# dojo-sim/ContactImplicitMPC.jl

Hardware: AMD Instinct MI355X
Metric: MPC steps/s (quadruped, H=40, fp64) (higher is better)
Workload: dtype f64

## Files before the change

contactimplicitmpc/jl_amd/csrc/cimpc_host.cpp:

```cpp
#include <hip/hip_runtime.h>

#include <algorithm>
#include <chrono>
#include <cmath>
#include <cstdio>
#include <cstdlib>
#include <cstring>
#include <string>
#include <vector>

#include "cimpc_internal.h"
#include "lin_table.h"
#include "newton_state.h"
#include "schedule_plan.h"

using namespace cimpc;

namespace {

thread_local std::string g_create_error;

enum ProfClass { PC_IP = 0, PC_KKT = 1, PC_RESID = 2, PC_OTHER = 3, PC_ASYNC = 4, PC_COUNT = 5 };

struct ProfRec {
// ... 220 lines not shown
    (void)hipStreamSynchronize(h->stream);
    if (h->rs.st) (void)hipStreamSynchronize(h->rs.st);
    if (h->rs.st_kkt) (void)hipStreamSynchronize(h->rs.st_kkt);
    for (auto& r : h->prof_recs) {
        float ms = 0.f;
        if (hipEventElapsedTime(&ms, r.a, r.b) == hipSuccess) {
            h->prof_ms[r.cls] += ms;
            h->prof_n[r.cls] += 1;
        }
        h->ev_pool.push_back(r.a);
        h->ev_pool.push_back(r.b);
    }
    h->prof_recs.clear();
}

IpParams make_ip_params(cimpc_ctx* h, const TrajDev& T, int par, int* pending_counter, double* zout) {
    IpParams p{};
    p.tab = h->d_tab;
    p.Q = h->Q;
    p.Q.par = par;
    p.wpk = h->sched.wpk;
    p.q = T.q;
    p.theta = T.th;
    p.gam = T.g;
    p.bfr = T.b;
    p.alt = h->alt_set ? h->d_alt : nullptr;
    p.d = h->S.d;
    p.dz = h->S.dz;
    p.nu = nullptr; p.dtn = nullptr; p.dtn_ld = h->S.dtn_ld;
    p.status = h->S.ip_status;
    p.iters = h->S.ip_iters;
    p.zout = zout;
    p.pflag = h->S.pflag;
    p.pstate = h->d_pstate;
    p.pending_count = pending_counter;
    p.iter_cap = h->kn.sched.iter_cap;
    p.slots = CS;
    p.H = h->dm.H;
    p.o = h->ip;
    p.kc_floor = h->ip.kappa_tol / h->ip.undercut;
    p.tau_floor = 1.0 - h->ip.eps_min;
    p.reg_floor = h->ip.kappa_tol * h->ip.gamma_reg;
    p.budget_ticks = h->ip_budget_ticks;
    p.generic_static = h->kn.generic_static ? 1 : 0;
    return p;
}

int run_sweep(cimpc_ctx* h, int par, int* pending_counter, double* zout, hipStream_t st, int iter_cap = 0, int* drain_counter = nullptr,
              bool with_products = false, long long hint = -1) {
    IpParams p = make_ip_params(h, h->S.cand, par, pending_counter, zout);
    if (with_products && h->S.dtn != nullptr) { p.nu = h->S.nu_cand; p.dtn = h->S.dtn; }
    if (iter_cap > 0) p.iter_cap = iter_cap;
    const SweepLaunch l = plan_sweep(h->kn.sched, h->sched, hint, p.iter_cap, h->ip.max_iter, drain_counter != nullptr);
    p.wpk = l.wpk; p.direct = l.direct;
    if (l.drain_thresh > 0) { p.drain_count = drain_counter; p.drain_thresh = l.drain_thresh; p.drain_min = h->kn.sched.drain_min; }
    prof_begin(h, PC_IP, st);
    int rc = launch_ip_sweep(&h->dm, p, l.waves, st);
    prof_end(h, st);
    if (rc != CIMPC_OK) return fail(h, rc, "ip sweep launch failed");
    return CIMPC_OK;
}

static void set_kkt_backend(cimpc_ctx* h) {
    NewtonDev& S = h->S;
    KktCaps& c = h->kc;
    c.cfg = h->dm.mode == CIMPC_MODE_CONFIGURATION;
    c.velocity = S.V != nullptr;
    c.cf_tiny = h->cf_tiny;
    c.wide_tiles = (h->dm.nq > 16 || h->dm.nu > 16) && h->dm.nq <= 24 && h->dm.nu <= 24;
    c.condensed = kkt_condensed_available(S);
    c.mfma = kkt_mfma_available(S);
    c.packed = kkt_packed_available(S);
    c.twisted = kkt_twisted_available(S);
    c.duo = kkt_duo_available(S);
    c.mixed = kkt_mixed_available(S);
    auto pick_band_form = [&](auto avail) {
        for (int r = h->band_reduce_ok ? 1 : 0; r >= 0; --r) { S.band_reduce = r; if (avail()) return true; }
        S.band_reduce = h->band_reduce_ok ? 1 : 0;
        return false;
    };
    S.band_reduce = h->band_reduce_ok ? 1 : 0;
    c.banded = c.cfg && pick_band_form([&] { return kkt_banded_available(S); });
    c.cf_reduce = !c.cfg && (c.velocity ? pick_band_form([&] { return kkt_cf_reduce_available(S); }) : kkt_cf_reduce_available(S));
    c.banded_twisted = kkt_banded_twisted_available(c.cfg ? S : cf_shadow(S));
    h->kb = select_kkt_backend(c, h->nt.kkt_backend);
    S.good_src = kkt_lazy_commit(h->kp, c, h->kb) ? h->d_good_src : nullptr;
}

int ensure_kkt_ws(cimpc_ctx* h) {
    if (h->kb == KktBackend::Condensed) return CIMPC_OK;
    if (h->kb == KktBackend::CondensedMixed) {
        if (h->d_mix_ws) return CIMPC_OK;
        if (dev_alloc(h, &h->d_mix_ws, kkt_mixed_workspace_doubles(h->S)) != CIMPC_OK) return CIMPC_ERR_HIP;
        return dev_alloc(h, &h->d_mix_nfb, 1);
    }
    const bool cf = h->kb == KktBackend::CfCondensed || h->kb == KktBackend::CfBanded;
    if (cf && !h->d_cf_ws && dev_alloc(h, &h->d_cf_ws, cf_reduce_doubles(h->S)) != CIMPC_OK) return CIMPC_ERR_HIP;
    if (h->kb == KktBackend::CfCondensed) return CIMPC_OK;
    const size_t need = cf ? kkt_dense_workspace_doubles(cf_shadow(h->S), true) : kkt_dense_workspace_doubles(h->S, h->kb == KktBackend::Banded);
    if (h->d_dense_ws && h->dense_ws_doubles >= need) return CIMPC_OK;
    h->d_dense_ws = nullptr;
    h->dense_ws_doubles = need;
    return dev_alloc(h, &h->d_dense_ws, need);
}

static KktForm plan_kkt_stage(cimpc_ctx* h, const KktSite& site) {
    const KktForm f = choose_kkt_form(h->kp, h->kc, h->kb, site);
// ... 1248 lines not shown
```

contactimplicitmpc/jl_amd/csrc/cimpc_internal.h:

```cpp
#pragma once
#include <hip/hip_runtime.h>
#include <stdint.h>

#include "../../../include/cimpc.h"

namespace cimpc {

constexpr int QPAD = 32;
constexpr int CPAD = 32;

struct IpQueues {
    int* items;
    int* count;
    int* head;
    int* done_count;
    const int* window;
    int cap, K, par;
};

struct AsyncQ {
    int on;
    int* rq_items;
    int* rq_head;
    int* rq_tail;
// ... 60 lines not shown
    atomicAdd(A.epoch + 32 * 16, 1);
    atomicAdd(A.epoch + (16 + (b & 15)) * 16, 1);
}
__device__ __forceinline__ void push_kkt_job(const AsyncQ& A, int b) {
    if (A.kkt_tw) {
        const int pos = atomicAdd(A.kq_tail, 2);
        astore(A.kq_items + pos, b | (2 << KJOB_SHIFT));
        astore(A.kq_items + pos + 1, b | (1 << KJOB_SHIFT));
        atomicAdd(A.epoch + 32 * 16, 1);
        atomicAdd(A.epoch + (16 + (b & 15)) * 16, 1);
        atomicAdd(A.epoch + (16 + ((b + 1) & 15)) * 16, 1);
    } else {
        aq_push(A.kq_items, A.kq_tail, b);
        wake_job(A, b);
    }
}
__device__ __forceinline__ void wake_all(const AsyncQ& A) { for (int k = 0; k <= 32; ++k) atomicAdd(A.epoch + k * 16, 1); }

__device__ __forceinline__ int* qcount(const IpQueues& Q, int par, int k) { return Q.count + ((size_t)par * Q.K + k) * QPAD; }
__device__ __forceinline__ int* qhead(const IpQueues& Q, int k) { return Q.head + (size_t)k * QPAD; }

struct IpParams {
    const double* tab;
    IpQueues Q;
    int wpk;
    const double* q;
    const double* theta;
    const double* gam;
    const double* bfr;
    const double* alt;
    double* d;
    double* dz;
    const double* nu;
    double* dtn;
    int dtn_ld;
    int* status;
    int* iters;
    double* zout;
    int* pflag;
    double* pstate;
    int* pending_count;
    int iter_cap;
    int* drain_count;
    int drain_thresh, drain_min;
    int slots;
    int H;
    cimpc_ip_opts o;
    double kc_floor;
    double tau_floor;
    double reg_floor;
    long long budget_ticks;
    int generic_static;
    int direct;
    AsyncQ A;
};

struct IpCallbackArgs {
    const double* tab;
    int knot, n, op;
    const double* z;
    const double* theta;
    const double* alt;
    const double* r;
    double kappa, reg;
    double* out;
};

struct KernelInfo {
    int G;
    int lds_table;
    int lds_group;
    int tab_size;
    int dtn_ld;
    int adj;
    int generic;
};

struct LdsOptIn { size_t set[16] = {0}; };
inline int lds_opt_in(LdsOptIn& cache, const void* kernel, size_t lds) {
    if (lds <= 64 * 1024) return CIMPC_OK;
    int dev = 0;
    if (hipGetDevice(&dev) != hipSuccess) return CIMPC_ERR_HIP;
    dev &= 15;
    if (lds <= cache.set[dev]) return CIMPC_OK;
    if (hipFuncSetAttribute(kernel, hipFuncAttributeMaxDynamicSharedMemorySize, (int)lds) != hipSuccess) return CIMPC_ERR_HIP;
    cache.set[dev] = lds;
    return CIMPC_OK;
}
template <class Kern, class... Args>
int launch_lds(LdsOptIn& cache, Kern kernel, dim3 grid, dim3 block, size_t lds, hipStream_t s, Args... args) {
    if (lds_opt_in(cache, (const void*)kernel, lds) != CIMPC_OK) return CIMPC_ERR_HIP;
    hipLaunchKernelGGL(kernel, grid, block, lds, s, args...);
    return hipGetLastError() == hipSuccess ? CIMPC_OK : CIMPC_ERR_HIP;
}

int ip_kernel_info(const cimpc_dims* dm, KernelInfo* info);
int launch_ip_sweep(const cimpc_dims* dm, const IpParams& p, int waves, hipStream_t s);
int launch_ip_callback(const cimpc_dims* dm, const IpCallbackArgs& a, hipStream_t s);
bool ip_generic_available(const cimpc_dims* dm);
void ip_generic_info(const cimpc_dims* dm, KernelInfo* info);
int launch_ip_generic(const cimpc_dims* dm, const IpParams& p, hipStream_t s);

}
```

contactimplicitmpc/jl_amd/csrc/ip_kernel_impl.h:

```cpp
#pragma once
#include "cimpc_internal.h"
#include "lane_group.h"
#include "lin_table.h"

#define CIMPC_SWEEP_PRIO 0

namespace cimpc {

#ifdef CIMPC_SWEEP_PROF
static __device__ unsigned long long g_sweep_prof[16];
#define SPROF_T() ((long long)__builtin_amdgcn_s_memtime())
#else
#define SPROF_T() 0ll
#endif

template <int NQ_, int NU_, int NW_, int NC_, int NB_, int MODE_, int WIDE_ = 0>
struct Model {
    static constexpr int NQ = NQ_, NU = NU_, NW = NW_, NC = NC_, NB = NB_, MODE = MODE_;
    static constexpr bool WIDE = WIDE_ != 0;
    using Wide = Model<NQ_, NU_, NW_, NC_, NB_, MODE_, 1>;
    static constexpr int NX = NQ, NY = 2 * NC + NB, NZ = NQ + 4 * NC + 2 * NB;
    static constexpr int NTH = 2 * NQ + NU + NW + 2, NTHS = 2 * NQ + NU;
    static constexpr int ND = MODE ? NQ + NC + NB : NQ;
    static constexpr int G = (NX <= 16 && NY <= 16) ? 16 : (NX <= 32 && NY <= 32) ? 32 : 64;
    static_assert(NX <= 64 && NY <= 64, "lane group holds at most 64 rows");
    static constexpr bool FULL_TILE = !(WIDE && !(NX <= 16 && NY <= 16)) && G != 64;
    static constexpr int RROWS = FULL_TILE ? NY : 8;
    static constexpr int RST_LD = FULL_TILE ? G + 1 : G + 2;
    static constexpr int DTN_LD = ((NTHS + G - 1) / G) * G;
#ifndef CIMPC_SENS_ADJOINT
#define CIMPC_SENS_ADJOINT 1
#endif
    static constexpr int ADJ = (CIMPC_SENS_ADJOINT && MODE == 0) ? 1 : 0;
#define CIMPC_SENS_MAX 16
    static constexpr int SENS_MAX = CIMPC_SENS_MAX;
#define CIMPC_SENS_ILP 5
#ifndef CIMPC_SENS_ILP32
#define CIMPC_SENS_ILP32 3
#endif
    static constexpr int SENS_ILP = (NX <= 16 && NY <= 16) ? CIMPC_SENS_ILP : CIMPC_SENS_ILP32;
    static constexpr bool RLDS = !FULL_TILE && ADJ != 0;
    static_assert(G != 64 || RLDS, "64-lane groups: :configuration mode only (the adjoint sensitivity pass keeps the tile free for R)");
    static constexpr int RTRI = NY * (NY - 1) / 2;
    static constexpr int TILE0 = RLDS ? RTRI : RROWS * RST_LD;
    static constexpr int TILE = TILE0 > NTH ? TILE0 : NTH;
    static constexpr int OFF_BV = ((TILE + SENS_MAX / 2 + 1) + 1) & ~1;
#ifndef CIMPC_ADJ_ILP32
#define CIMPC_ADJ_ILP32 3
#endif
#ifndef CIMPC_ADJ_CB
#define CIMPC_ADJ_CB 4
#endif
#ifndef CIMPC_ADJ_ILP64
#define CIMPC_ADJ_ILP64 3
#endif
#ifndef CIMPC_ADJ_CB64
#define CIMPC_ADJ_CB64 2
#endif
    static constexpr int ADJ_ILP = (NX <= 16 && NY <= 16) ? 4 : G == 64 ? CIMPC_ADJ_ILP64 : CIMPC_ADJ_ILP32;
    static constexpr int NBV0 = CIMPC_SENS_ILP32 > 3 ? CIMPC_SENS_ILP32 : 3;
    static constexpr int NBV = (ADJ && ADJ_ILP > NBV0) ? ADJ_ILP : NBV0;
    static constexpr int BVEC = (G == 16) ? 0 : NBV * G;
    static constexpr int LDS_GROUP = OFF_BV + BVEC;
};

__device__ __forceinline__ void wave_lds_fence() {
    __builtin_amdgcn_fence(__ATOMIC_ACQ_REL, "wavefront");
    __builtin_amdgcn_wave_barrier();
}

template <class M>
struct IpSolver {
    static constexpr int NX = M::NX, NY = M::NY, NTH = M::NTH, G = M::G;
    static constexpr LinLayout L{NX, NY, NTH, G, M::NTHS, M::ADJ};
    using LG = LaneGroup<G>;

    const double* tab;
    const double* ctab;
    double* Rst;
    double* bv;
    int l;
    int csl;
    bool vx, vy;
    double ry2, ry1d, caibd, rdyn0, rrst0, x0, y10, y20;
    double tthdyn, tthrst, altl;
    double x, y1, y2, rdyn, rrst, rbil, Dx_, Dy1_, Dy2_;
    double Qc[NY], Rr[NY], rdinv, y1r, y2r, iy1r;

    __device__ __forceinline__ void bind(const double* tab_, double* Rst_, int l_, const double* ctab_ = nullptr) {
        tab = tab_; Rst = Rst_; l = l_;
        ctab = ctab_ != nullptr ? ctab_ : tab_;
        bv = Rst_ + M::OFF_BV;
        csl = l_ * (l_ - 1) / 2;
        vx = l < NX; vy = l < NY;
        const double* tVec = tab + L.oVecL;
        ry2 = tVec[LinLayout::V_RY2 * G + l];
        ry1d = tVec[LinLayout::V_RY1D * G + l];
        caibd = tVec[LinLayout::V_CAIBD * G + l];
        rdyn0 = tVec[LinLayout::V_RDYN0 * G + l];
        rrst0 = tVec[LinLayout::V_RRST0 * G + l];
        x0 = tVec[LinLayout::V_X0 * G + l];
        y10 = tVec[LinLayout::V_Y10 * G + l];
        y20 = tVec[LinLayout::V_Y20 * G + l];
        rdinv = 0.0; y1r = y2r = iy1r = 1.0;
        tthdyn = tthrst = altl = 0.0;
    }

    __device__ __forceinline__ void stage(double v) const {
        wave_lds_fence();
        bv[l] = v;
        wave_lds_fence();
    }

    __device__ __forceinline__ void spread32(double v, double& c0, double& c1) const {
        const unsigned lo = (unsigned)__double2loint(v), hi = (unsigned)__double2hiint(v);
        const auto r0 = __builtin_amdgcn_permlane16_swap(lo, lo, false, false);
        const auto r1 = __builtin_amdgcn_permlane16_swap(hi, hi, false, false);
        c0 = __hiloint2double((int)r1[0], (int)r0[0]);
        c1 = __hiloint2double((int)r1[1], (int)r0[1]);
    }
    template <int N, class TF>
// ... 631 lines not shown
            if constexpr (M::MODE == CIMPC_MODE_CONFIGURATIONFORCE)
                static_for<0, NC + NB>([&](auto kc) { constexpr int k = decltype(kc)::value; s_ = fma(col[NX + k], LG::template bcast<k>(nuy), s_); });
            if (l < n) xst<ASYNC>(p.dtn + pi * (size_t)M::DTN_LD + c0 + lg, s_);
            wave_lds_fence();
        }
    }
    problem_done<ASYNC>(p, prob / p.H, l, part == 0);
}

#define CIMPC_PICK_MAXK 256
constexpr int PICK_MAXK = CIMPC_PICK_MAXK;
__device__ __forceinline__ int pick_knot(const IpParams& p, int* s_rem, int* s_total, int* s_knot, int tid, int wg, int nwg) {
    const int K = p.Q.K, par = p.Q.par;
    if (tid == 0) *s_total = 0;
    __syncthreads();
    {
        int part = 0;
        for (int k = tid; k < K; k += (int)blockDim.x) {
            int rem = aload(qcount(p.Q, par, k)) - aload(qhead(p.Q, k));
            rem = rem > 0 ? rem : 0;
            if (k < PICK_MAXK) s_rem[k] = rem;
            part += rem;
        }
        if (part > 0) atomicAdd(s_total, part);
    }
    __syncthreads();
    if (tid == 0) {
        const int total = *s_total;
        int pick = -1;
        if (total > 0) {
            const long long target = ((long long)wg * total) / (long long)nwg;
            long long acc = 0;
            for (int k = 0; k < K; ++k) {
                const int rem = k < PICK_MAXK ? s_rem[k] : max(0, aload(qcount(p.Q, par, k)) - aload(qhead(p.Q, k)));
                if (rem > 0) { pick = k; acc += rem; if (acc > target) break; }
            }
        }
        *s_knot = pick;
    }
    __syncthreads();
    return *s_knot;
}

template <class M, bool ASYNC>
__device__ __forceinline__ void serve_knot(const IpParams& p, double* smem, int knot, int tid, [[maybe_unused]] long long* sp = nullptr) {
    constexpr int NX = M::NX, NY = M::NY, NTH = M::NTH, ND = M::ND, G = M::G;
    constexpr int NC = M::NC, NB = M::NB;
    constexpr LinLayout L(NX, NY, NTH, G, M::NTHS, M::ADJ);
    constexpr int PS = 2 * NX + 4 * NY + 4;
    double* tab = smem;
    const int K = p.Q.K, cap = p.Q.cap, par = p.Q.par;
    const int grp = tid / G;
    const int l = tid % G;
    double* Rst = smem + L.hot + (size_t)grp * M::LDS_GROUP;
    double* dth = Rst;
    constexpr int GPW = 64 / G;
    static_assert(M::SENS_MAX >= 2 * GPW, "the wave's list holds a trip's worth of problems plus one trip of new arrivals");
    const int gw = (tid & 63) / G;
    int* backlog = reinterpret_cast<int*>(smem + L.hot + (size_t)(grp - gw) * M::LDS_GROUP + M::TILE);
    int nback = 0;
    const bool vx = l < NX, vy = l < NY;
    const cimpc_ip_opts o = p.o;
    long long* tbase = reinterpret_cast<long long*>(smem + L.hot + (size_t)grp * M::LDS_GROUP + M::TILE + M::SENS_MAX / 2);
    const bool timed = p.budget_ticks > 0;

    [[maybe_unused]] const long long sp_t0 = SPROF_T();
    const int n = ASYNC ? 1 : *qcount(p.Q, par, knot);
    stage_table<M>(tab, p.tab, knot, tid);
    __syncthreads();
#ifdef CIMPC_SWEEP_PROF
    if (sp) sp[2] += SPROF_T() - sp_t0;
#endif
    const int* items = p.Q.items + ((size_t)par * K + knot) * cap;
    int* head = qhead(p.Q, knot);
    [[maybe_unused]] const int* tailp = qcount(p.Q, par, knot);
    IpSolver<M> S;
    const double* ctab = (L.hot == L.size) ? tab : p.tab + (size_t)knot * L.size;
    S.bind(tab, Rst, l, ctab);
    bool have = false, exhausted = false, stalled = false;
    int prob = 0, iters = 0, done_here = 0;
    [[maybe_unused]] int idle_trips = 0, dbg_trips = 0, dbg_act = 0;
    [[maybe_unused]] long long dbg_tpop = 0, dbg_tfence = 0;
    [[maybe_unused]] long long dbg_pop[4] = {0, 0, 0, 0};
    [[maybe_unused]] const bool dbg_on = ASYNC && p.A.dbg != nullptr;
    double reg = 0.0, r_vio = 0.0, k_vio = 0.0, qinit = 0.0;
    [[maybe_unused]] int drain_raw = 0;

    while (true) {
        [[maybe_unused]] const long long sp_a = SPROF_T();
        [[maybe_unused]] bool draining = false;
        int lg = l;
        asm volatile("" : "+v"(lg));
        if constexpr (!ASYNC) {
            if (p.drain_count != nullptr) {
                draining = __builtin_amdgcn_readfirstlane(drain_raw) >= p.drain_thresh;
                drain_raw = aload(p.drain_count);
            }
        }
        bool push = false;
        long long t_used = 0;
        if (timed) t_used = (long long)wall_clock64() - *tbase;
        if (have) {
            int code = -1;
            if (stalled) code = 0;
            else if (r_vio < o.r_tol && k_vio < o.kappa_tol) code = 1;
            else if (iters >= o.max_iter || (timed && t_used >= p.budget_ticks)) code = 0;
            else if (done_here >= p.iter_cap || (!ASYNC && draining && done_here >= p.drain_min)) code = 2;
            if (code >= 0) {
                const size_t pi = (size_t)prob;
                const int sb = prob / p.H;
                double* ps = p.pstate + pi * PS;
                if (code == 2) {
                    if (vx) { ps[lg] = S.x; ps[NX + 2 * NY + lg] = S.rdyn; }
                    if (vy) { ps[NX + lg] = S.y1; ps[NX + NY + lg] = S.y2; ps[2 * NX + 2 * NY + lg] = S.rrst; ps[2 * NX + 3 * NY + lg] = S.rbil; }
                    if (l == 0) {
                        ps[PS - 4] = r_vio; ps[PS - 3] = k_vio; ps[PS - 2] = reg; ps[PS - 1] = (double)((long long)iters + (timed ? t_used * 128 : 0));
                        p.pflag[pi] = 1;
                        const int pos = atomicAdd(qcount(p.Q, par ^ 1, knot), 1);
                        p.Q.items[((size_t)(par ^ 1) * K + knot) * cap + pos] = prob;
                        atomicAdd(p.pending_count, 1);
                    }
                } else {
                    if (l == 0) { xst<ASYNC>(p.status + pi, code); xst<ASYNC>(p.iters + pi, iters); }
                    if (vx) xst<ASYNC>(p.d + pi * ND + lg, S.x - qinit);
                    if constexpr (M::MODE == CIMPC_MODE_CONFIGURATIONFORCE) {
                        if (l < NC) xst<ASYNC>(p.d + pi * ND + NX + lg, S.y1 - xld<ASYNC>(p.gam + pi * NC + lg));
                        else if (l < NC + NB) xst<ASYNC>(p.d + pi * ND + NX + lg, S.y1 - xld<ASYNC>(p.bfr + pi * NB + (lg - NC)));
                    }
                    if (p.zout != nullptr) {
                        double* zo = p.zout + pi * M::NZ;
                        if (vx) zo[lg] = S.x;
                        if (vy) { zo[NX + lg] = S.y1; zo[NX + NY + lg] = S.y2; }
                    }
                    if (code == 1) {
                        if (vx) ps[lg] = S.x;
                        if (vy) { ps[NX + lg] = S.y1; ps[NX + NY + lg] = S.y2; }
                        if (l == 0) ps[PS - 2] = reg;
                        push = true;
                    } else {
                        {
                            const long long t0 = dbg_on ? wall_clock64() : 0;
                            problem_done<ASYNC>(p, sb, l);
                            if (dbg_on) dbg_tfence += wall_clock64() - t0;
                        }
                    }
                }
                have = false;
            }
        }
        {
            const unsigned long long pm = __ballot((push && l == 0) ? 1 : 0);
            if (pm != 0ull) {
                if (push && l == 0) backlog[nback + __popcll(pm & ((1ull << (tid & 63)) - 1ull))] = prob;
                nback += __popcll(pm);
            }
        }
        [[maybe_unused]] const long long sp_b = SPROF_T();
        if (!have && (!exhausted || (ASYNC && (++idle_trips & 7) == 0))) {
            int idx = 0, item = 0;
            if constexpr (ASYNC) {
                const long long tq0 = dbg_on ? wall_clock64() : 0;
                if (l == 0) item = aq_pop(const_cast<int*>(items), head, tailp, p.A.dbg ? dbg_pop : nullptr, p.A.abort_flag);
                item = group_bcast0<G>(item);
                idx = item < 0 ? n : 0;
                const long long tq1 = dbg_on ? wall_clock64() : 0;
                if (item >= 0) xfence(p.A.flags);
                if (dbg_on) { dbg_tpop += tq1 - tq0; dbg_tfence += wall_clock64() - tq1; }
            } else {
                if (l == 0) idx = atomicAdd(head, 1);
                idx = group_bcast0<G>(idx);
            }
            if (idx < n) {
                prob = ASYNC ? item : items[idx];
                const int sb = prob / p.H, i = prob - sb * p.H;
                const size_t pi = (size_t)prob;
                const double* th = p.theta + pi * NTH;
                constexpr int NTC = (NTH + G - 1) / G;
                double thv[NTC];
                static_for<0, NTC>([&](auto jc) {
                    constexpr int j = decltype(jc)::value;
                    const int k = lg + j * G;
                    thv[j] = xld<ASYNC>(th + (k < NTH ? k : 0));
                });
                const double alt_in = (p.alt != nullptr && l < NC) ? p.alt[(size_t)(sb / p.slots) * NC + lg] : 0.0;
                const double* qrow = p.q + ((size_t)sb * (p.H + 2) + (i + 2)) * M::NQ;
                const double q_in = vx ? xld<ASYNC>(qrow + lg) : 0.0;
                const int parked_in = p.pflag[pi];
                static_for<0, NTC>([&](auto jc) {
                    constexpr int j = decltype(jc)::value;
                    const int k = l + j * G;
                    if (k < NTH) dth[k] = thv[j] - ctab[L.oTh0 + k];
                });
                wave_lds_fence();
                {
                    double a0 = 0.0, a1 = 0.0, c0 = 0.0, c1 = 0.0;
                    if constexpr (G == 16) {
                        constexpr int CHK = 8;
                        static_for<0, (NTH + CHK - 1) / CHK>([&](auto cc) {
                            constexpr int k0 = decltype(cc)::value * CHK, n = NTH - k0 < CHK ? NTH - k0 : CHK;
                            double dv[n], od[n], orr[n];
                            static_for<0, n>([&](auto jc) {
                                constexpr int j = decltype(jc)::value;
                                dv[j] = dth[k0 + j]; od[j] = ctab[L.oRthDyn + (k0 + j) * G + l]; orr[j] = ctab[L.oRthRst + (k0 + j) * G + l];
                            });
                            pin_values(dv); pin_values(od); pin_values(orr);
                            static_for<0, n>([&](auto jc) {
                                constexpr int j = decltype(jc)::value;
                                if constexpr (((k0 + j) & 1) == 0) { a0 = fma(od[j], dv[j], a0); c0 = fma(orr[j], dv[j], c0); }
                                else { a1 = fma(od[j], dv[j], a1); c1 = fma(orr[j], dv[j], c1); }
                            });
                        });
                    } else {
                        int k = 0;
                        for (; k + 1 < NTH; k += 2) {
                            const double d0 = dth[k], d1 = dth[k + 1];
                            a0 = fma(ctab[L.oRthDyn + k * G + l], d0, a0);
                            c0 = fma(ctab[L.oRthRst + k * G + l], d0, c0);
                            a1 = fma(ctab[L.oRthDyn + (k + 1) * G + l], d1, a1);
                            c1 = fma(ctab[L.oRthRst + (k + 1) * G + l], d1, c1);
                        }
                        for (; k < NTH; ++k) {
                            const double d0 = dth[k];
                            a0 = fma(ctab[L.oRthDyn + k * G + l], d0, a0);
                            c0 = fma(ctab[L.oRthRst + k * G + l], d0, c0);
                        }
                    }
                    S.tthdyn = a0 + a1;
                    S.tthrst = c0 + c1;
                }
                S.altl = alt_in;
                qinit = q_in;
                const double* ps = p.pstate + pi * PS;
                if (parked_in == 1) {
                    S.x = vx ? ps[lg] : 0.0;
                    S.y1 = vy ? ps[NX + lg] : 1.0;
                    S.y2 = vy ? ps[NX + NY + lg] : 1.0;
                    S.rdyn = vx ? ps[NX + 2 * NY + lg] : 0.0;
                    S.rrst = vy ? ps[2 * NX + 2 * NY + lg] : 0.0;
                    S.rbil = vy ? ps[2 * NX + 3 * NY + lg] : 0.0;
                    r_vio = ps[PS - 4]; k_vio = ps[PS - 3]; reg = ps[PS - 2];
                    const long long it_word = (long long)ps[PS - 1];
                    iters = timed ? (int)(it_word & 127) : (int)it_word;
                    if (timed && l == 0) *tbase = (long long)wall_clock64() - (it_word >> 7);
                    wave_lds_fence();
                    if (l == 0) p.pflag[pi] = 0;
                } else {
                    S.x = qinit; S.y1 = 1.0; S.y2 = 1.0;
                    S.residual(0.0);
                    r_vio = S.r_violation();
                    k_vio = S.k_violation();
                    iters = 0;
                    reg = 0.0;
                    if (timed && l == 0) *tbase = (long long)wall_clock64();
                }
                if (timed) wave_lds_fence();
                done_here = 0;
                stalled = false;
                have = true;
#ifdef CIMPC_SWEEP_PROF
                if (sp) sp[8] += 1;
#endif
            } else {
                exhausted = true;
            }
        }
        [[maybe_unused]] const long long sp_c = SPROF_T();
#ifdef CIMPC_SWEEP_PROF
        if (sp) { sp[3] += sp_b - sp_a; sp[4] += sp_c - sp_b; }
#endif
        if (dbg_on) { dbg_trips += 1; dbg_act += have ? 1 : 0; }
        const bool any_ip = __any(have ? 1 : 0);
        if (!any_ip && nback == 0) break;
        const bool sens_trip = !any_ip || nback >= GPW || (ASYNC && nback > 0 && __any(have ? 0 : 1));
        if (!sens_trip) {
            if (have && !(r_vio < o.r_tol && k_vio < o.kappa_tol) && iters < o.max_iter && done_here < p.iter_cap) {
                ++done_here;
                ++iters;
                stalled = S.iterate(o, p.kc_floor, p.tau_floor, reg, r_vio, k_vio);
            }
        } else {
            int take, part = 0, nparts = 1;
            if (nback >= GPW) { take = nback - 1 - gw; nback -= GPW; }
            else {
                if (nback == 1) { take = 0; part = gw; nparts = GPW; }
                else if (GPW == 4 && nback == 2) { take = gw >> 1; part = gw & 1; nparts = 2; }
                else take = gw < nback ? gw : -1;
                nback = 0;
            }
            wave_lds_fence();
            if (take >= 0) {
                const double sx = S.x, sy1 = S.y1, sy2 = S.y2, sd = S.rdyn, sr = S.rrst, sb_ = S.rbil, st = S.tthdyn, su = S.tthrst, sa = S.altl;
                const int pr = backlog[take];
                sensitivities<M, ASYNC>(p, S, tab, pr, l, part, nparts);
                S.x = sx; S.y1 = sy1; S.y2 = sy2; S.rdyn = sd; S.rrst = sr; S.rbil = sb_; S.tthdyn = st; S.tthrst = su; S.altl = sa;
            }
        }
#ifdef CIMPC_SWEEP_PROF
        if (sp) { const long long sp_d = SPROF_T(); if (sens_trip) { sp[6] += sp_d - sp_c; sp[10] += 1; } else { sp[5] += sp_d - sp_c; sp[9] += 1; } }
#endif
    }
    if constexpr (ASYNC) {
        if (p.A.dbg != nullptr && l == 0) {
            atomicAdd((unsigned long long*)p.A.dbg + 4, (unsigned long long)dbg_act);
            atomicAdd((unsigned long long*)p.A.dbg + 5, (unsigned long long)dbg_trips);
            atomicAdd((unsigned long long*)p.A.dbg + 6, (unsigned long long)dbg_tpop);
            atomicAdd((unsigned long long*)p.A.dbg + 7, (unsigned long long)dbg_tfence);
            for (int k = 0; k < 4; ++k) atomicAdd((unsigned long long*)p.A.dbg + 12 + k, (unsigned long long)dbg_pop[k]);
        }
    }
}

#define CIMPC_SWEEP_OCC 2
#define CIMPC_SWEEP_THREADS 256
template <class M>
__global__ __launch_bounds__(M::G == 16 ? CIMPC_SWEEP_THREADS : (M::WIDE ? 512 : 256), M::G == 16 ? CIMPC_SWEEP_OCC : 1) void ip_queue_kernel(IpParams p) {
    extern __shared__ __attribute__((aligned(16))) double smem[];
    __shared__ int s_knot, s_total, s_rem[PICK_MAXK];
    const int tid = (int)threadIdx.x;
    __builtin_amdgcn_s_setprio(CIMPC_SWEEP_PRIO);
    [[maybe_unused]] long long sp[12] = {0, 0, 0, 0, 0, 0, 0, 0, 0, 0, 0, 0};
    [[maybe_unused]] const long long sp_life = SPROF_T();
    if (p.direct) {
        const int knot = (int)blockIdx.x;
        if (knot < p.Q.K && aload(qcount(p.Q, p.Q.par, knot)) > 0) serve_knot<M, false>(p, smem, knot, tid, sp);
        return;
    }
    while (true) {
        [[maybe_unused]] const long long sp_t = SPROF_T();
        __syncthreads();
        const int knot = pick_knot(p, s_rem, &s_total, &s_knot, tid, (int)blockIdx.x, (int)gridDim.x);
#ifdef CIMPC_SWEEP_PROF
        sp[1] += SPROF_T() - sp_t;
#endif
        if (knot < 0) {
            if (tid == 0 && p.drain_count != nullptr) atomicAdd(p.drain_count, 1);
            break;
        }
        serve_knot<M, false>(p, smem, knot, tid, sp);
    }
#ifdef CIMPC_SWEEP_PROF
    if ((tid & 63) == 0) {
        sp[0] = SPROF_T() - sp_life; sp[7] = 1;
        for (int k = 0; k < 11; ++k) atomicAdd(&g_sweep_prof[k], (unsigned long long)sp[k]);
    }
#endif
}

template <class M>
__global__ __launch_bounds__(64) void ip_callback_kernel(IpCallbackArgs a) {
    constexpr int NX = M::NX, NY = M::NY, NTH = M::NTH, G = M::G;
    constexpr LinLayout L(NX, NY, NTH, G, M::NTHS, M::ADJ);
    extern __shared__ __attribute__((aligned(16))) double smem[];
    const int tid = (int)threadIdx.x, grp = tid / G, l = tid % G;
    double* tab = smem;
    double* Rst = smem + L.size + (size_t)grp * M::LDS_GROUP;
    stage_table<M>(tab, a.tab, a.knot, tid);
    __syncthreads();
    const int prob = (int)blockIdx.x * (64 / G) + grp;
    const bool live = prob < a.n;
    const size_t pi = (size_t)(live ? prob : 0);
    IpSolver<M> S;
    S.bind(tab, Rst, l);
    const bool vx = S.vx, vy = S.vy;
    const double* z = a.z + pi * M::NZ;
    S.x = vx ? z[l] : 0.0;
    S.y1 = vy ? z[NX + l] : 1.0;
    S.y2 = vy ? z[NX + NY + l] : 1.0;
    double* out = a.out + pi * M::NZ;
    if (a.op == 0) {
        const double* th = a.theta + pi * NTH;
        double td[2] = {0.0, 0.0}, tr[2] = {0.0, 0.0};
        for (int k = 0; k < NTH; ++k) {
            const double dk = th[k] - tab[L.oTh0 + k];
            td[k & 1] = fma(tab[L.oRthDyn + k * G + l], dk, td[k & 1]);
            tr[k & 1] = fma(tab[L.oRthRst + k * G + l], dk, tr[k & 1]);
        }
        S.tthdyn = td[0] + td[1]; S.tthrst = tr[0] + tr[1];
        S.altl = (a.alt != nullptr && l < M::NC) ? a.alt[pi * M::NC + l] : 0.0;
        S.residual(a.kappa);
        if (live && vx) out[l] = S.rdyn;
        if (live && vy) { out[NX + l] = S.rrst; out[NX + NY + l] = S.rbil; }
    } else {
        const double* r = a.r + pi * M::NZ;
        S.rdyn = vx ? r[l] : 0.0;
        S.rrst = vy ? r[NX + l] : 0.0;
        S.rbil = vy ? r[NX + NY + l] : 0.0;
        S.factorize(a.reg);
        S.linear_solve();
        if (live && vx) out[l] = S.Dx_;
        if (live && vy) { out[NX + l] = S.Dy1_; out[NX + NY + l] = S.Dy2_; }
    }
}

template <class M>
int launch_callback(const IpCallbackArgs& a, hipStream_t s) {
    constexpr LinLayout L(M::NX, M::NY, M::NTH, M::G, M::NTHS, M::ADJ);
    const int ppw = 64 / M::G;
    const size_t lds = (size_t)(L.size + ppw * M::LDS_GROUP) * sizeof(double);
    static LdsOptIn optin;
    if (lds_opt_in(optin, (const void*)ip_callback_kernel<M>, lds) != CIMPC_OK) return CIMPC_ERR_HIP;
    hipLaunchKernelGGL((ip_callback_kernel<M>), dim3((a.n + ppw - 1) / ppw), dim3(64), lds, s, a);
    return hipGetLastError() == hipSuccess ? CIMPC_OK : CIMPC_ERR_HIP;
}

template <class M>
int launch_model(const IpParams& p, int waves, hipStream_t s) {
    constexpr LinLayout L(M::NX, M::NY, M::NTH, M::G, M::NTHS, M::ADJ);
    if (waves < 1 || waves > (M::G == 16 ? CIMPC_SWEEP_THREADS : 512) / 64 || waves == 3) return CIMPC_ERR_INVALID;
    const int ppw = 64 / M::G;
    const size_t lds = (size_t)(L.hot + waves * ppw * M::LDS_GROUP) * sizeof(double);
    const int grid = p.wpk;
    if constexpr (M::G == 64) { if (waves > 4) return CIMPC_ERR_INVALID; }
    if constexpr (M::G == 32) {
        if (waves > 4) {
            using MW = typename M::Wide;
            constexpr LinLayout LW(MW::NX, MW::NY, MW::NTH, MW::G, MW::NTHS, MW::ADJ);
            const size_t lds_w = (size_t)(LW.size + waves * ppw * MW::LDS_GROUP) * sizeof(double);
            static LdsOptIn optin_w;
            if (lds_opt_in(optin_w, (const void*)ip_queue_kernel<MW>, lds_w) != CIMPC_OK) return CIMPC_ERR_HIP;
            hipLaunchKernelGGL((ip_queue_kernel<MW>), dim3(grid), dim3(64 * waves), lds_w, s, p);
            return hipGetLastError() == hipSuccess ? CIMPC_OK : CIMPC_ERR_HIP;
        }
    }
    static LdsOptIn optin;
    if (lds_opt_in(optin, (const void*)ip_queue_kernel<M>, lds) != CIMPC_OK) return CIMPC_ERR_HIP;
    hipLaunchKernelGGL((ip_queue_kernel<M>), dim3(grid), dim3(64 * waves), lds, s, p);
    return hipGetLastError() == hipSuccess ? CIMPC_OK : CIMPC_ERR_HIP;
}

template <class M>
void info_model(KernelInfo* info) {
    constexpr LinLayout L(M::NX, M::NY, M::NTH, M::G, M::NTHS, M::ADJ);
    info->G = M::G;
    info->lds_table = L.hot;
    info->lds_group = M::LDS_GROUP;
    info->tab_size = L.size;
    info->dtn_ld = M::DTN_LD;
    info->adj = M::ADJ;
}

#define CIMPC_DEFINE_MODEL(name, q, u, w, c, b)                                              \
    int ip_launch_##name(int mode, const IpParams& p, int waves, hipStream_t s) {            \
        if (mode == 0) return launch_model<Model<q, u, w, c, b, 0>>(p, waves, s);            \
        return launch_model<Model<q, u, w, c, b, 1>>(p, waves, s);                           \
    }                                                                                        \
    int ip_callback_##name(int mode, const IpCallbackArgs& a, hipStream_t s) {               \
        if (mode == 0) return launch_callback<Model<q, u, w, c, b, 0>>(a, s);                \
        return launch_callback<Model<q, u, w, c, b, 1>>(a, s);                               \
    }                                                                                        \
    void ip_info_##name(int mode, KernelInfo* info) {                                        \
        if (mode == 0) info_model<Model<q, u, w, c, b, 0>>(info);                            \
        else info_model<Model<q, u, w, c, b, 1>>(info);                                      \
    }

#define CIMPC_DEFINE_MODEL64(name, q, u, w, c, b)                                            \
    int ip_launch_##name(int mode, const IpParams& p, int waves, hipStream_t s) {            \
        if (mode != 0) return CIMPC_ERR_INVALID;                                             \
        return launch_model<Model<q, u, w, c, b, 0>>(p, waves, s);                           \
    }                                                                                        \
    void ip_info_##name(int mode, KernelInfo* info) { (void)mode; info_model<Model<q, u, w, c, b, 0>>(info); }

}

#ifdef CIMPC_UBENCH
// ... 50 lines not shown
```

contactimplicitmpc/jl_amd/csrc/schedule_plan.h:

```cpp
#pragma once
#include <algorithm>
#include <cstddef>
#include "kkt_plan.h"

namespace cimpc {

struct SchedulePolicy {
    int async_mode = 2;
    int async_tail = -1;
    int async_full_max = 32;
    int spec_first = -1;
    int iter_cap = 28;
    int tail_div = 8;
    int drain_pct = 95;
    int drain_min = 4;
    int sweep_wgs = 0;
    int waves32 = 0;
};
struct ScheduleFacts {
    int B = 1, H = 1, H_ref = 1, G = 16;
    bool async_available = false;
};
struct SchedulePlan {
    ScheduleFacts f;
// ... 9 lines not shown
constexpr int async_idle_sleep = 2, async_idle_spins = 48, async_wake_fan = 1;

inline SchedulePlan plan_schedule(const SchedulePolicy& p, const ScheduleFacts& f) {
    SchedulePlan s;
    const int B = (s.f = f).B;
    s.async_on = p.async_mode != 0 && f.async_available;
    s.single_launch = s.async_on && (p.async_mode == 1 || (p.async_mode == 2 && B >= 4 && B <= p.async_full_max));
    s.hybrid = s.async_on && p.async_mode == 2 && !s.single_launch && B > p.async_full_max;
    s.async_tail = p.async_tail >= 0 ? p.async_tail : f.G == 32 ? 16 : B < 256 ? std::max(32, B / 4) : std::min(96, std::max(64, B / 6));
    s.spec_all = B <= 128 ? 3 : 8;
    s.spec_first = p.spec_first >= 0 ? p.spec_first : (B <= 1024 ? 3 : 1);
    s.spec_mid = B > 128 ? 1 : 8;
    s.kkt_overlap = B >= 64;
    if (f.G == 32) {
        if (p.waves32 > 0 && p.waves32 < 1000) s.waves = p.waves32;
        else if ((size_t)B * f.H >= 6000) s.waves = 8;
        s.adapt32 = p.waves32 >= 1000 ? p.waves32 : (p.waves32 == 4 || p.waves32 == 8) ? 0 : 7000;
    }
    if (s.single_launch) s.waves = 4;
    const size_t groups_per_wg = (64 / f.G) * s.waves;
    const size_t nprob = (size_t)B * f.H;
    size_t w = (nprob + 2 * groups_per_wg - 1) / (2 * groups_per_wg);
    w = std::max<size_t>(w, std::min<size_t>(f.H_ref, nprob));
    const size_t resident = (size_t)256 * std::max(1, (f.G == 16 ? (s.waves > 4 ? 2 * s.waves : 8) : 4) / s.waves);
    s.wpk = p.sweep_wgs > 0 ? p.sweep_wgs : (int)std::max<size_t>(1, std::min<size_t>(w, resident));
    const int a_wgs = p.sweep_wgs > 0 ? s.wpk : std::max(s.wpk, 240);
    s.async_service = std::max(1, a_wgs / 8);
    s.async_grid = std::max((int)std::min<size_t>(resident, (size_t)a_wgs + s.async_service), s.async_service + 1);
    const int tail = std::max(256, 3 * s.async_tail);
    s.tail_grid = std::min(tail, s.async_grid);
    s.tail_service = tail < s.async_grid ? std::max(1, tail / 8) : s.async_service;
    return s;
}

enum class SolvePath { Rounds, Persistent, Hybrid };
inline SolvePath choose_solve_path(const SchedulePlan& s, KktBackend be) {
    return be != KktBackend::Condensed ? SolvePath::Rounds : s.single_launch ? SolvePath::Persistent : s.hybrid ? SolvePath::Hybrid : SolvePath::Rounds;
}
inline int max_rounds(const SchedulePolicy& p, int newton_max_iter, int ip_max_iter) {
    const int min_progress = p.drain_pct > 0 ? std::min(p.iter_cap, p.drain_min) : p.iter_cap;
    return (newton_max_iter * 8 + 2) * ((ip_max_iter + min_progress - 1) / min_progress + 1);
}

inline bool round_ahead(const SchedulePlan& s, KktBackend be, bool warm_start, bool budget) { return s.f.B < 4 && be != KktBackend::CondensedMixed && warm_start && !budget; }
struct RoundPlan { int cap, n_slots; bool split_join; };
inline RoundPlan plan_round(const SchedulePolicy& p, const SchedulePlan& s, int ip_max_iter, bool kkt, bool blind, int last_sweep, int last_slots) {
    const bool sparse = p.tail_div > 0 && (s.f.B < p.tail_div || (!blind && (long long)last_sweep * p.tail_div <= s.f.B));
    const int cap = sparse ? ip_max_iter : p.iter_cap;
    const int n_slots = s.kkt_overlap ? last_slots : (s.f.B < 4 ? -2 : -1);
    return {cap, n_slots, kkt && s.kkt_overlap && n_slots >= 0};
}

inline bool hand_over(const SchedulePlan& s, int active) { return active > 0 && active <= s.async_tail; }
struct SweepLaunch { int waves, wpk; bool direct; int drain_thresh; };
inline SweepLaunch plan_sweep(const SchedulePolicy& p, const SchedulePlan& s, long long hint, int iter_cap, int ip_max_iter, bool drain) {
    SweepLaunch l{s.waves, s.wpk, false, 0};
    if (s.adapt32 > 0 && hint > 0 && s.kkt_overlap && p.sweep_wgs <= 0) {
        l.waves = hint >= s.adapt32 ? 8 : 4;
        const size_t groups_per_wg = 2 * (size_t)l.waves;
        size_t w = ((size_t)hint + 2 * groups_per_wg - 1) / (2 * groups_per_wg);
        w = std::max<size_t>(w, std::min<size_t>((size_t)s.f.H_ref, (size_t)std::max<long long>(hint, 1)));
        l.wpk = (int)std::max<size_t>(1, std::min<size_t>(w, 256));
    }
    if (s.f.B < 4 && p.sweep_wgs <= 0) { l.direct = true; l.wpk = s.f.H_ref; }
    if (drain && p.drain_pct > 0 && iter_cap < ip_max_iter) l.drain_thresh = std::max(1, (int)((long long)l.wpk * p.drain_pct / 100));
    return l;
}

}
```

Before: 73380.

## Add claim-ahead prefetch of next sweep item into an LDS stash via DMA

Adds a per-wave LDS stash and a small claim state machine to the IP sweep kernel. While a group is still solving its current problem, it reserves the next queue index and pulls that problem's theta, q, alt and parked flag into LDS with global_load_lds. The aim is to hide the global-load latency of picking up new work. The feature is gated by a guard computed on the host, and a constexpr switch currently leaves that guard at zero. Even so, the stash LDS, the extra wave fences and the changed drain-counter load still run in the G=16 configuration-mode variant, which may cost occupancy and add per-trip overhead.

```diff
diff --git a/contactimplicitmpc/jl_amd/csrc/cimpc_host.cpp b/contactimplicitmpc/jl_amd/csrc/cimpc_host.cpp
--- a/contactimplicitmpc/jl_amd/csrc/cimpc_host.cpp
+++ b/contactimplicitmpc/jl_amd/csrc/cimpc_host.cpp
@@ -296,7 +296,7 @@
     if (with_products && h->S.dtn != nullptr) { p.nu = h->S.nu_cand; p.dtn = h->S.dtn; }
     if (iter_cap > 0) p.iter_cap = iter_cap;
     const SweepLaunch l = plan_sweep(h->kn.sched, h->sched, hint, p.iter_cap, h->ip.max_iter, drain_counter != nullptr);
-    p.wpk = l.wpk; p.direct = l.direct;
+    p.wpk = l.wpk; p.direct = l.direct; p.guard = l.guard;
     if (l.drain_thresh > 0) { p.drain_count = drain_counter; p.drain_thresh = l.drain_thresh; p.drain_min = h->kn.sched.drain_min; }
     prof_begin(h, PC_IP, st);
     int rc = launch_ip_sweep(&h->dm, p, l.waves, st);
diff --git a/contactimplicitmpc/jl_amd/csrc/cimpc_internal.h b/contactimplicitmpc/jl_amd/csrc/cimpc_internal.h
--- a/contactimplicitmpc/jl_amd/csrc/cimpc_internal.h
+++ b/contactimplicitmpc/jl_amd/csrc/cimpc_internal.h
@@ -136,6 +136,7 @@
     long long budget_ticks;
     int generic_static;
     int direct;
+    int guard;
     AsyncQ A;
 };
 
diff --git a/contactimplicitmpc/jl_amd/csrc/ip_kernel_impl.h b/contactimplicitmpc/jl_amd/csrc/ip_kernel_impl.h
--- a/contactimplicitmpc/jl_amd/csrc/ip_kernel_impl.h
+++ b/contactimplicitmpc/jl_amd/csrc/ip_kernel_impl.h
@@ -2,6 +2,7 @@
 #include "cimpc_internal.h"
 #include "lane_group.h"
 #include "lin_table.h"
+#include "sweep_claim.h"
 
 #define CIMPC_SWEEP_PRIO 0
 
@@ -62,11 +63,28 @@
     static constexpr int NBV = (ADJ && ADJ_ILP > NBV0) ? ADJ_ILP : NBV0;
     static constexpr int BVEC = (G == 16) ? 0 : NBV * G;
     static constexpr int LDS_GROUP = OFF_BV + BVEC;
+    static constexpr int STASH_W = 2 * (NTH + NX + NC) + 1;
+    static constexpr int STASH_SLOTS = (STASH_W + 15) / 16 + 1;
+    static constexpr int STASH_WAVE = (G == 16 && MODE == 0) ? STASH_SLOTS * 32 : 0;
+    static constexpr int STASH_WG = 4 * STASH_WAVE;
 };
 
 __device__ __forceinline__ void wave_lds_fence() {
     __builtin_amdgcn_fence(__ATOMIC_ACQ_REL, "wavefront");
     __builtin_amdgcn_wave_barrier();
+}
+
+__device__ __forceinline__ void lds_dma_word(const void* g, unsigned lds_base) {
+    unsigned keep;
+    asm volatile("s_mov_b32 %0, m0\n\ts_mov_b32 m0, %2\n\ts_nop 0\n\tglobal_load_lds_dword %1, off\n\ts_mov_b32 m0, %0\n\ts_nop 0"
+                 : "=&s"(keep) : "v"(g), "s"(lds_base) : "memory");
+}
+__device__ __forceinline__ void lds_dma_wait() {
+    __builtin_amdgcn_s_waitcnt(0x0F70);
+    asm volatile("" ::: "memory");
+}
+__device__ __forceinline__ unsigned lds_byte_address(const void* p) {
+    return (unsigned)(unsigned long long)(__attribute__((address_space(3))) const void*)p;
 }
 
 template <class M>
@@ -804,16 +822,18 @@
     const int K = p.Q.K, cap = p.Q.cap, par = p.Q.par;
     const int grp = tid / G;
     const int l = tid % G;
-    double* Rst = smem + L.hot + (size_t)grp * M::LDS_GROUP;
+    constexpr bool PF = !ASYNC && G == 16 && M::MODE == CIMPC_MODE_CONFIGURATION;
+    constexpr int goff = L.hot + (PF ? M::STASH_WG : 0);
+    double* Rst = smem + goff + (size_t)grp * M::LDS_GROUP;
     double* dth = Rst;
     constexpr int GPW = 64 / G;
     static_assert(M::SENS_MAX >= 2 * GPW, "the wave's list holds a trip's worth of problems plus one trip of new arrivals");
     const int gw = (tid & 63) / G;
-    int* backlog = reinterpret_cast<int*>(smem + L.hot + (size_t)(grp - gw) * M::LDS_GROUP + M::TILE);
+    int* backlog = reinterpret_cast<int*>(smem + goff + (size_t)(grp - gw) * M::LDS_GROUP + M::TILE);
     int nback = 0;
     const bool vx = l < NX, vy = l < NY;
     const cimpc_ip_opts o = p.o;
-    long long* tbase = reinterpret_cast<long long*>(smem + L.hot + (size_t)grp * M::LDS_GROUP + M::TILE + M::SENS_MAX / 2);
+    long long* tbase = reinterpret_cast<long long*>(smem + goff + (size_t)grp * M::LDS_GROUP + M::TILE + M::SENS_MAX / 2);
     const bool timed = p.budget_ticks > 0;
 
     [[maybe_unused]] const long long sp_t0 = SPROF_T();
@@ -837,19 +857,71 @@
     [[maybe_unused]] const bool dbg_on = ASYNC && p.A.dbg != nullptr;
     double reg = 0.0, r_vio = 0.0, k_vio = 0.0, qinit = 0.0;
     [[maybe_unused]] int drain_raw = 0;
+    constexpr int SI = (M::STASH_SLOTS - 1) * 64;
+    [[maybe_unused]] int pf_got = 0;
+    if constexpr (PF) {
+        int* st0 = reinterpret_cast<int*>(smem + L.hot + (size_t)(tid >> 6) * M::STASH_WAVE) + gw * 16;
+        if (l == 0) st0[SI + 2] = CLAIM_NONE;
+        wave_lds_fence();
+    }
 
     while (true) {
         [[maybe_unused]] const long long sp_a = SPROF_T();
         [[maybe_unused]] bool draining = false;
         int lg = l;
         asm volatile("" : "+v"(lg));
+        [[maybe_unused]] int* stash = nullptr;
+        [[maybe_unused]] unsigned stash_lds = 0;
+        [[maybe_unused]] int ev = 0;
+        if constexpr (PF) {
+            int tg = tid;
+            asm volatile("" : "+v"(tg));
+            double* sw = smem + L.hot + (size_t)(tg >> 6) * M::STASH_WAVE;
+            stash = reinterpret_cast<int*>(sw) + ((tg & 63) / G) * 16;
+            stash_lds = (unsigned)__builtin_amdgcn_readfirstlane((int)lds_byte_address(sw));
+        }
+        [[maybe_unused]] int pf = CLAIM_NONE;
+        if constexpr (PF) pf = stash[SI + 2];
         if constexpr (!ASYNC) {
             if (p.drain_count != nullptr) {
                 draining = __builtin_amdgcn_readfirstlane(drain_raw) >= p.drain_thresh;
-                drain_raw = aload(p.drain_count);
-            }
+                if constexpr (!PF) drain_raw = aload(p.drain_count);
+            }
+        }
+        if constexpr (PF) {
+            if (pf == CLAIM_INDEX) {
+                const int got = group_bcast0<G>(pf_got);
+                if (claim_returned(pf, exhausted, got, n)) {
+                    if (l == 0) { stash[SI + 1] = got; lds_dma_word(items + got, stash_lds + (unsigned)(SI * 4)); }
+                } else ev |= 4;
+            } else if (pf == CLAIM_ITEM) {
+                lds_dma_wait();
+                const int nprob = stash[SI];
+                const int sb = nprob / p.H, i = nprob - sb * p.H;
+                const size_t pi = (size_t)nprob;
+                const int* thw = reinterpret_cast<const int*>(p.theta + pi * NTH);
+                const int* qw = reinterpret_cast<const int*>(p.q + ((size_t)sb * (p.H + 2) + (i + 2)) * M::NQ);
+                const int* aw = p.alt != nullptr ? reinterpret_cast<const int*>(p.alt + (size_t)(sb / p.slots) * NC) : thw;
+                static_for<0, M::STASH_SLOTS - 1>([&](auto kc) {
+                    constexpr int k = decltype(kc)::value, lo = 16 * k, hi = lo + 16, W0 = 2 * NTH, W1 = W0 + 2 * NX, W2 = W1 + 2 * NC;
+                    const int w = lo + lg;
+                    const int* src = thw;
+                    if constexpr (lo < W0) src = (hi <= W0 || w < W0) ? thw + w : src;
+                    if constexpr (hi > W0 && lo < W1) src = ((lo >= W0 || w >= W0) && (hi <= W1 || w < W1)) ? qw + (w - W0) : src;
+                    if constexpr (hi > W1 && lo < W2) src = ((lo >= W1 || w >= W1) && (hi <= W2 || w < W2)) ? aw + (w - W1) : src;
+                    if constexpr (hi > W2 && lo <= W2) src = w == W2 ? p.pflag + pi : src;
+                    lds_dma_word(src, stash_lds + (unsigned)(k * 256));
+                });
+                claim_item_arrived(pf);
+            } else if (pf == CLAIM_INPUT) {
+                lds_dma_wait();
+                claim_input_arrived(pf);
+            }
+            wave_lds_fence();
+            if (p.drain_count != nullptr) drain_raw = aload(p.drain_count);
         }
         bool push = false;
+        int push_prob = 0;
         long long t_used = 0;
         if (timed) t_used = (long long)wall_clock64() - *tbase;
         if (have) {
@@ -859,6 +931,7 @@
             else if (iters >= o.max_iter || (timed && t_used >= p.budget_ticks)) code = 0;
             else if (done_here >= p.iter_cap || (!ASYNC && draining && done_here >= p.drain_min)) code = 2;
             if (code >= 0) {
+                if constexpr (PF) prob = stash[SI + 3];
                 const size_t pi = (size_t)prob;
                 const int sb = prob / p.H;
                 double* ps = p.pstate + pi * PS;
@@ -889,6 +962,7 @@
                         if (vy) { ps[NX + lg] = S.y1; ps[NX + NY + lg] = S.y2; }
                         if (l == 0) ps[PS - 2] = reg;
                         push = true;
+                        push_prob = prob;
                     } else {
                         {
                             const long long t0 = dbg_on ? wall_clock64() : 0;
@@ -903,13 +977,16 @@
         {
             const unsigned long long pm = __ballot((push && l == 0) ? 1 : 0);
             if (pm != 0ull) {
-                if (push && l == 0) backlog[nback + __popcll(pm & ((1ull << (tid & 63)) - 1ull))] = prob;
+                if (push && l == 0) backlog[nback + __popcll(pm & ((1ull << (tid & 63)) - 1ull))] = push_prob;
                 nback += __popcll(pm);
             }
         }
         [[maybe_unused]] const long long sp_b = SPROF_T();
-        if (!have && (!exhausted || (ASYNC && (++idle_trips & 7) == 0))) {
+        [[maybe_unused]] int pk = PULL_DEMAND;
+        if constexpr (PF) pk = pull_kind(pf, exhausted);
+        if (!have && (PF ? pk != PULL_WAIT : (!exhausted || (ASYNC && (++idle_trips & 7) == 0)))) {
             int idx = 0, item = 0;
+            const bool from_stash = PF && pk == PULL_STASH;
             if constexpr (ASYNC) {
                 const long long tq0 = dbg_on ? wall_clock64() : 0;
                 if (l == 0) item = aq_pop(const_cast<int*>(items), head, tailp, p.A.dbg ? dbg_pop : nullptr, p.A.abort_flag);
@@ -918,26 +995,53 @@
                 const long long tq1 = dbg_on ? wall_clock64() : 0;
                 if (item >= 0) xfence(p.A.flags);
                 if (dbg_on) { dbg_tpop += tq1 - tq0; dbg_tfence += wall_clock64() - tq1; }
+            } else if (from_stash) {
+                idx = stash[SI + 1];
+                item = stash[SI];
             } else {
                 if (l == 0) idx = atomicAdd(head, 1);
                 idx = group_bcast0<G>(idx);
+                if constexpr (PF) {
+                    if (idx < n) { item = items[idx]; asm volatile("" : "+v"(item)); }
+                }
             }
             if (idx < n) {
-                prob = ASYNC ? item : items[idx];
+                prob = (ASYNC || PF) ? item : items[idx];
                 const int sb = prob / p.H, i = prob - sb * p.H;
                 const size_t pi = (size_t)prob;
                 const double* th = p.theta + pi * NTH;
                 constexpr int NTC = (NTH + G - 1) / G;
-                double thv[NTC];
-                static_for<0, NTC>([&](auto jc) {
-                    constexpr int j = decltype(jc)::value;
-                    const int k = lg + j * G;
-                    thv[j] = xld<ASYNC>(th + (k < NTH ? k : 0));
-                });
-                const double alt_in = (p.alt != nullptr && l < NC) ? p.alt[(size_t)(sb / p.slots) * NC + lg] : 0.0;
-                const double* qrow = p.q + ((size_t)sb * (p.H + 2) + (i + 2)) * M::NQ;
-                const double q_in = vx ? xld<ASYNC>(qrow + lg) : 0.0;
-                const int parked_in = p.pflag[pi];
+                double thv[NTC], alt_in, q_in;
+                int parked_in;
+                if (from_stash) {
+                    const double* sd = reinterpret_cast<const double*>(stash);
+                    static_for<0, NTC>([&](auto jc) {
+                        constexpr int j = decltype(jc)::value;
+                        const int k = l + j * G < NTH ? l + j * G : 0;
+                        thv[j] = sd[(k >> 3) * 32 + (k & 7)];
+                    });
+                    const int kq = NTH + l, ka = NTH + NX + l;
+                    q_in = vx ? sd[(kq >> 3) * 32 + (kq & 7)] : 0.0;
+                    alt_in = (p.alt != nullptr && l < NC) ? sd[(ka >> 3) * 32 + (ka & 7)] : 0.0;
+                    parked_in = stash[((M::STASH_W - 1) / 16) * 64 + (M::STASH_W - 1) % 16];
+                    claim_taken(pf);
+                    ev |= 1;
+                } else {
+                    static_for<0, NTC>([&](auto jc) {
+                        constexpr int j = decltype(jc)::value;
+                        const int k = lg + j * G;
+                        thv[j] = xld<ASYNC>(th + (k < NTH ? k : 0));
+                    });
+                    alt_in = (p.alt != nullptr && l < NC) ? p.alt[(size_t)(sb / p.slots) * NC + lg] : 0.0;
+                    const double* qrow = p.q + ((size_t)sb * (p.H + 2) + (i + 2)) * M::NQ;
+                    q_in = vx ? xld<ASYNC>(qrow + lg) : 0.0;
+                    parked_in = p.pflag[pi];
+                    if constexpr (PF) {
+                        pin_values(thv);
+                        asm volatile("" : "+v"(alt_in), "+v"(q_in), "+v"(parked_in));
+                    }
+                    ev |= 2;
+                }
                 static_for<0, NTC>([&](auto jc) {
                     constexpr int j = decltype(jc)::value;
                     const int k = l + j * G;
@@ -993,6 +1097,7 @@
                     r_vio = ps[PS - 4]; k_vio = ps[PS - 3]; reg = ps[PS - 2];
                     const long long it_word = (long long)ps[PS - 1];
                     iters = timed ? (int)(it_word & 127) : (int)it_word;
+                    asm volatile("" : "+v"(S.x), "+v"(S.y1), "+v"(S.y2), "+v"(S.rdyn), "+v"(S.rrst), "+v"(S.rbil), "+v"(r_vio), "+v"(k_vio), "+v"(reg), "+v"(iters));
                     if (timed && l == 0) *tbase = (long long)wall_clock64() - (it_word >> 7);
                     wave_lds_fence();
                     if (l == 0) p.pflag[pi] = 0;
@@ -1009,20 +1114,41 @@
                 done_here = 0;
                 stalled = false;
                 have = true;
+                if constexpr (PF) {
+                    if (l == 0) stash[SI + 3] = prob;
+                    if (claim_on_take(pf, exhausted, p.guard, n, idx)) {
+                        int zero = 0;
+                        asm volatile("" : "+v"(zero));
+                        if (l == 0) pf_got = atomicAdd(head + zero, 1);
+                    }
+                }
 #ifdef CIMPC_SWEEP_PROF
                 if (sp) sp[8] += 1;
 #endif
             } else {
                 exhausted = true;
+                ev |= 4;
             }
         }
         [[maybe_unused]] const long long sp_c = SPROF_T();
 #ifdef CIMPC_SWEEP_PROF
-        if (sp) { sp[3] += sp_b - sp_a; sp[4] += sp_c - sp_b; }
+        if (sp) {
+            sp[3] += sp_b - sp_a; sp[4] += sp_c - sp_b;
+            sp[12] += __any((ev & 3) ? 1 : 0) ? 1 : 0;
+            sp[13] += __popcll(__ballot(((ev & 4) && l == 0) ? 1 : 0));
+            sp[14] += __popcll(__ballot(((ev & 1) && l == 0) ? 1 : 0));
+            sp[15] += __popcll(__ballot(((ev & 2) && l == 0) ? 1 : 0));
+        }
 #endif
         if (dbg_on) { dbg_trips += 1; dbg_act += have ? 1 : 0; }
         const bool any_ip = __any(have ? 1 : 0);
-        if (!any_ip && nback == 0) break;
+        bool claims = false;
+        if constexpr (PF) {
+            if (l == 0) stash[SI + 2] = pf;
+            wave_lds_fence();
+            claims = __any(claim_pending(pf) ? 1 : 0);
+        }
+        if (!any_ip && nback == 0 && !claims) break;
         const bool sens_trip = !any_ip || nback >= GPW || (ASYNC && nback > 0 && __any(have ? 0 : 1));
         if (!sens_trip) {
             if (have && !(r_vio < o.r_tol && k_vio < o.kappa_tol) && iters < o.max_iter && done_here < p.iter_cap) {
@@ -1046,6 +1172,7 @@
                 sensitivities<M, ASYNC>(p, S, tab, pr, l, part, nparts);
                 S.x = sx; S.y1 = sy1; S.y2 = sy2; S.rdyn = sd; S.rrst = sr; S.rbil = sb_; S.tthdyn = st; S.tthrst = su; S.altl = sa;
             }
+            if constexpr (PF) lds_dma_wait();
         }
 #ifdef CIMPC_SWEEP_PROF
         if (sp) { const long long sp_d = SPROF_T(); if (sens_trip) { sp[6] += sp_d - sp_c; sp[10] += 1; } else { sp[5] += sp_d - sp_c; sp[9] += 1; } }
@@ -1070,7 +1197,7 @@
     __shared__ int s_knot, s_total, s_rem[PICK_MAXK];
     const int tid = (int)threadIdx.x;
     __builtin_amdgcn_s_setprio(CIMPC_SWEEP_PRIO);
-    [[maybe_unused]] long long sp[12] = {0, 0, 0, 0, 0, 0, 0, 0, 0, 0, 0, 0};
+    [[maybe_unused]] long long sp[16] = {0, 0, 0, 0, 0, 0, 0, 0, 0, 0, 0, 0, 0, 0, 0, 0};
     [[maybe_unused]] const long long sp_life = SPROF_T();
     if (p.direct) {
         const int knot = (int)blockIdx.x;
@@ -1088,12 +1215,13 @@
             if (tid == 0 && p.drain_count != nullptr) atomicAdd(p.drain_count, 1);
             break;
         }
+        if (tid < 64) sp[11] += 1;
         serve_knot<M, false>(p, smem, knot, tid, sp);
     }
 #ifdef CIMPC_SWEEP_PROF
     if ((tid & 63) == 0) {
         sp[0] = SPROF_T() - sp_life; sp[7] = 1;
-        for (int k = 0; k < 11; ++k) atomicAdd(&g_sweep_prof[k], (unsigned long long)sp[k]);
+        for (int k = 0; k < 16; ++k) atomicAdd(&g_sweep_prof[k], (unsigned long long)sp[k]);
     }
 #endif
 }
@@ -1160,8 +1288,9 @@
     constexpr LinLayout L(M::NX, M::NY, M::NTH, M::G, M::NTHS, M::ADJ);
     if (waves < 1 || waves > (M::G == 16 ? CIMPC_SWEEP_THREADS : 512) / 64 || waves == 3) return CIMPC_ERR_INVALID;
     const int ppw = 64 / M::G;
-    const size_t lds = (size_t)(L.hot + waves * ppw * M::LDS_GROUP) * sizeof(double);
+    const size_t lds = (size_t)(L.hot + waves * ppw * M::LDS_GROUP + M::STASH_WG) * sizeof(double);
     const int grid = p.wpk;
+    static_assert(M::STASH_WG == 0 || M::STASH_WG == (CIMPC_SWEEP_THREADS / 64) * M::STASH_WAVE, "the stash has room for every wave of the largest sweep workgroup");
     if constexpr (M::G == 64) { if (waves > 4) return CIMPC_ERR_INVALID; }
     if constexpr (M::G == 32) {
         if (waves > 4) {
diff --git a/contactimplicitmpc/jl_amd/csrc/schedule_plan.h b/contactimplicitmpc/jl_amd/csrc/schedule_plan.h
--- a/contactimplicitmpc/jl_amd/csrc/schedule_plan.h
+++ b/contactimplicitmpc/jl_amd/csrc/schedule_plan.h
@@ -85,7 +85,12 @@
 }
 
 inline bool hand_over(const SchedulePlan& s, int active) { return active > 0 && active <= s.async_tail; }
-struct SweepLaunch { int waves, wpk; bool direct; int drain_thresh; };
+struct SweepLaunch { int waves, wpk; bool direct; int drain_thresh; int guard = 0; };
+inline int sweep_guard(const ScheduleFacts& f, const SweepLaunch& l) {
+    if (f.G != 16 || f.B < 4 || l.direct) return 0;
+    return ((l.wpk + f.H_ref - 1) / std::max(1, f.H_ref)) * (64 / f.G) * l.waves;
+}
+constexpr bool sweep_claim_ahead = false;
 inline SweepLaunch plan_sweep(const SchedulePolicy& p, const SchedulePlan& s, long long hint, int iter_cap, int ip_max_iter, bool drain) {
     SweepLaunch l{s.waves, s.wpk, false, 0};
     if (s.adapt32 > 0 && hint > 0 && s.kkt_overlap && p.sweep_wgs <= 0) {
@@ -97,6 +102,7 @@
     }
     if (s.f.B < 4 && p.sweep_wgs <= 0) { l.direct = true; l.wpk = s.f.H_ref; }
     if (drain && p.drain_pct > 0 && iter_cap < ip_max_iter) l.drain_thresh = std::max(1, (int)((long long)l.wpk * p.drain_pct / 100));
+    if (sweep_claim_ahead) l.guard = sweep_guard(s.f, l);
     return l;
 }
 
diff --git a/contactimplicitmpc/jl_amd/csrc/sweep_claim.h b/contactimplicitmpc/jl_amd/csrc/sweep_claim.h
--- /dev/null
+++ b/contactimplicitmpc/jl_amd/csrc/sweep_claim.h
@@ -0,0 +1,40 @@
+#pragma once
+
+#if defined(__HIPCC__)
+#define CIMPC_CLAIM_FN __host__ __device__ __forceinline__
+#else
+#define CIMPC_CLAIM_FN inline
+#endif
+
+namespace cimpc {
+
+enum ClaimPhase : int { CLAIM_NONE = 0, CLAIM_INDEX = 1, CLAIM_ITEM = 2, CLAIM_INPUT = 3, CLAIM_READY = 4 };
+enum PullKind : int { PULL_WAIT = 0, PULL_STASH = 1, PULL_DEMAND = 2 };
+
+CIMPC_CLAIM_FN bool claim_ahead_allowed(int guard, int n, int idx) { return guard > 0 && n - idx > guard; }
+
+CIMPC_CLAIM_FN bool claim_on_take(int& phase, bool exhausted, int guard, int n, int idx) {
+    if (phase != CLAIM_NONE || exhausted || !claim_ahead_allowed(guard, n, idx)) return false;
+    phase = CLAIM_INDEX;
+    return true;
+}
+CIMPC_CLAIM_FN bool claim_returned(int& phase, bool& exhausted, int got, int n) {
+    if (got < n) { phase = CLAIM_ITEM; return true; }
+    phase = CLAIM_NONE;
+    exhausted = true;
+    return false;
+}
+CIMPC_CLAIM_FN void claim_item_arrived(int& phase) { phase = CLAIM_INPUT; }
+CIMPC_CLAIM_FN void claim_input_arrived(int& phase) { phase = CLAIM_READY; }
+CIMPC_CLAIM_FN int pull_kind(int phase, bool exhausted) {
+    return phase == CLAIM_READY ? PULL_STASH : (phase == CLAIM_NONE && !exhausted) ? PULL_DEMAND : PULL_WAIT;
+}
+CIMPC_CLAIM_FN void claim_taken(int& phase) { phase = CLAIM_NONE; }
+CIMPC_CLAIM_FN bool demand_returned(bool& exhausted, int got, int n) {
+    if (got < n) return true;
+    exhausted = true;
+    return false;
+}
+CIMPC_CLAIM_FN bool claim_pending(int phase) { return phase != CLAIM_NONE; }
+
+}
```

Result: slower. 70040 (-4.5%).
